# sp-nitech/diffsptk

Measured on AMD Instinct MI355X. Metric: frames/sec STFT->mcep (fl=400 fp=80 nfft=512 M=24), higher is better.
Workload: dtype f32; 1 GPU; BASELINE configs[4] per-GPU shard: STFT->mcep forward, 1024 utterances x 1 s @ 16 kHz per GPU (204800 frames), alpha=0.42 n_iter=10; N=8 is the full 8192-utterance batch; features all-gathered over RCCL when N>1; utterances_per_gpu=1024, global_batch=1024, parallelism=dp1, rccl_world_size=1, reserved_cus=0, gather_depth=0, streams=1

## Files before the change

### diffsptk_amd/csrc/f16_split.h

```cpp
#pragma once

#include "common.h"
#include "mcep_solve.h"

namespace dsa {

typedef _Float16 f16x8 __attribute__((ext_vector_type(8)));
typedef _Float16 f16x4 __attribute__((ext_vector_type(4)));
typedef float f32x2v __attribute__((ext_vector_type(2)));
typedef _Float16 f16x2 __attribute__((ext_vector_type(2)));
typedef const __attribute__((address_space(1))) f16x8* gf16x8_ptr;
typedef int i32x4v __attribute__((ext_vector_type(4)));
__device__ __forceinline__ __amdgpu_buffer_rsrc_t image_rsrc(const _Float16* base, int bytes)
{
    return __builtin_amdgcn_make_buffer_rsrc(const_cast<_Float16*>(base), 0, bytes, 0x00020000);
}
__device__ __forceinline__ f16x8 gload8(__amdgpu_buffer_rsrc_t rsrc, unsigned lane_bytes, int const_bytes)
{
    const i32x4v r = __builtin_amdgcn_raw_buffer_load_b128(rsrc, (int)lane_bytes, const_bytes, 0);
    return __builtin_bit_cast(f16x8, r);
}
typedef const __attribute__((address_space(1))) float* gf32_ptr;

namespace mh {
using namespace mm;
constexpr float SD = 16.f;
constexpr float SM = 1024.f;
constexpr float SE = 65536.f;
constexpr int SE_LOG2 = 16;
constexpr float SG = 4096.f;
constexpr float SL = 128.f;
constexpr int IMG_D = 16 * 64 * 8, IMG_E = 24 * 64 * 8, IMG_G = 16 * 64 * 8;
constexpr int IMG_DH = 0, IMG_DL = IMG_DH + IMG_D, IMG_EH = IMG_DL + IMG_D, IMG_EL = IMG_EH + IMG_E;
constexpr int IMG_GH = IMG_EL + IMG_E, IMG_GL = IMG_GH + IMG_G, IMG_HALVES = IMG_GL + IMG_G;
constexpr int IMG_BYTES = IMG_HALVES * 2 + 32 * 4;
constexpr int EMAX_LOG2 = 15;
constexpr int DH_OFF = 0;
constexpr int DL_OFF = DH_OFF + 16 * 64 * 4;
constexpr int EH_OFF = DL_OFF + 16 * 64 * 4;
constexpr int EL_OFF = EH_OFF + 24 * 64 * 4;
}

namespace mhb {
using namespace mh;
constexpr int IMG_EB = 16 * 2 * 64 * 8, IMG_DB = 2 * 8 * 64 * 8, IMG_GB = 16 * 64 * 8;
constexpr int B_BASE = IMG_BYTES / 2;
constexpr int IMG_EBH = B_BASE, IMG_EBL = IMG_EBH + IMG_EB;
constexpr int IMG_DBH = IMG_EBL + IMG_EB, IMG_DBL = IMG_DBH + IMG_DB;
constexpr int IMG_GBH = IMG_DBL + IMG_DB, IMG_GBL = IMG_GBH + IMG_GB;
constexpr int IMG_B_HALVES = IMG_GBL + IMG_GB;
constexpr int TAIL_B = 32 + 64 + 256;
constexpr int IMG_B_BYTES = IMG_B_HALVES * 2 + TAIL_B * 4;
}

namespace mrh {
constexpr int WAVES = 4;
constexpr int LOG2_SD = 9;
constexpr int LOG2_SE = 16;
constexpr int EMAX_LOG2 = 13;
constexpr int stage_halves(int ks1, int nt) { return (4 * ks1 + 2 * nt) * 512; }
}

__device__ __forceinline__ f32x4 mfma_h(f16x8 a, f16x8 b, f32x4 c)
{
    return __builtin_amdgcn_mfma_f32_16x16x32_f16(a, b, c, 0, 0, 0);
}

__device__ __forceinline__ void split2(float x0, float x1, f16x2& hi, f16x2& lo)
{
    hi = __builtin_convertvector(f32x2v{x0, x1}, f16x2);
    const unsigned hb = __builtin_bit_cast(unsigned, hi);
    unsigned lb;
    asm("v_fma_mixlo_f16 %0, %1, -1.0, %2 op_sel_hi:[1,0,0]\n\ts_nop 0\n\t"
        "v_fma_mixhi_f16 %0, %1, -1.0, %3 op_sel:[1,0,0] op_sel_hi:[1,0,0]\n\ts_nop 0"
        : "=&v"(lb) : "v"(hb), "v"(x0), "v"(x1));
    lo = __builtin_bit_cast(f16x2, lb);
}
__device__ __forceinline__ void split4(float x0, float x1, float x2, float x3, f16x2& hiA, f16x2& hiB, f16x2& loA, f16x2& loB)
{
    hiA = __builtin_convertvector(f32x2v{x0, x1}, f16x2);
    hiB = __builtin_convertvector(f32x2v{x2, x3}, f16x2);
    const unsigned ha = __builtin_bit_cast(unsigned, hiA), hb = __builtin_bit_cast(unsigned, hiB);
    unsigned la, lb;
    asm("v_fma_mixlo_f16 %0, %2, -1.0, %4 op_sel_hi:[1,0,0]\n\t"
        "v_fma_mixlo_f16 %1, %3, -1.0, %6 op_sel_hi:[1,0,0]\n\t"
        "v_fma_mixhi_f16 %0, %2, -1.0, %5 op_sel:[1,0,0] op_sel_hi:[1,0,0]\n\t"
        "v_fma_mixhi_f16 %1, %3, -1.0, %7 op_sel:[1,0,0] op_sel_hi:[1,0,0]\n\ts_nop 0"
        : "=&v"(la), "=&v"(lb) : "v"(ha), "v"(hb), "v"(x0), "v"(x1), "v"(x2), "v"(x3));
    loA = __builtin_bit_cast(f16x2, la);
    loB = __builtin_bit_cast(f16x2, lb);
}
#ifdef DSA_MCEP_NOPK
__device__ __forceinline__ f32x2v fma2(f32x2v c, float s, f32x2v b)
{
    float r0 = __builtin_fmaf(c[0], s, b[0]), r1 = __builtin_fmaf(c[1], s, b[1]);
    asm volatile("" : "+v"(r0));
    return f32x2v{r0, r1};
}
#else
__device__ __forceinline__ f32x2v fma2(f32x2v c, float s, f32x2v b) { return c * f32x2v{s, s} + b; }
#endif
__device__ __forceinline__ f32x2v lo2(f32x4 v) { return __builtin_shufflevector(v, v, 0, 1); }
__device__ __forceinline__ f32x2v hi2(f32x4 v) { return __builtin_shufflevector(v, v, 2, 3); }

__device__ __forceinline__ void split1(float x, _Float16& hi, _Float16& lo)
{
    hi = (_Float16)x;
    lo = (_Float16)(x - (float)hi);
}

__device__ __forceinline__ void split8(const float (&v)[8], f16x8& hi, f16x8& lo)
{
#pragma unroll
    for (int i = 0; i < 8; i += 2) {
        f16x2 h, l;
        split2(v[i], v[i + 1], h, l);
        hi[i] = h[0]; hi[i + 1] = h[1];
        lo[i] = l[0]; lo[i + 1] = l[1];
    }
}

}
```

### diffsptk_amd/csrc/mcep_mfma_f16.h

```cpp
#pragma once

#include <type_traits>

#include "common.h"
#include "f16_split.h"
#include "mcep_solve.h"
#include "pk_math.h"

namespace dsa {

struct StftIn {
    const float* x;
    long Tlen, N;
    int P, left;
    const float* w;
    const float* twiddle;
    float eps;
    float* X_out;
    int pad_mode;
    int zmean;
    float floor_lin;
};

namespace mh {
constexpr float STOP_TAU = 0x1p-20f;
constexpr float STOP_FACTOR = 16.f;
constexpr int H_UPREV = 56;
static_assert(H_UPREV > 48 && H_UPREV < RS, "u_prev sits in the unused tail of the frame's rt window");
constexpr int H_E48 = EL_OFF + 24 * 64 * 4;
constexpr int H_E256 = H_E48 + 256;
constexpr int H_D256 = H_E256 + 52;
constexpr int H_AV = H_D256 + 32;
constexpr int H_NAV = H_AV + 28;
constexpr int H_ZERO = H_NAV + 28;
constexpr int H_WAVE = H_ZERO + 28;
constexpr int h_lds_floats(int waves) { return H_WAVE + waves * WAVE_FLOATS; }
constexpr int FU_LC = 400;
constexpr int FU_NR = (FU_LC + 31) / 32;
constexpr int FU_S = 272;
constexpr int FU_T256 = 0;
constexpr int FU_WTAB = FU_T256 + 512;
constexpr int FU_TWS = FU_WTAB + 2 * 16 * FU_NR;
constexpr int FU_FLOATS = FU_TWS + 256;
static_assert(4 * 272 * 2 == WAVE_FLOATS, "a wave's rt / rr windows double as the STFT tile of four frames");
static_assert(FU_TWS % 4 == 0 && H_WAVE % 4 == 0 && WAVE_FLOATS % 4 == 0, "16-byte aligned LDS tables");
constexpr int h_lds_floats_fused(int waves) { return h_lds_floats(waves) + FU_FLOATS; }
}

#ifndef DSA_FUSED_PK_MASK
#define DSA_FUSED_PK_MASK 31
#endif
#ifndef DSA_FUSED_DBG
#define DSA_FUSED_DBG 0
#endif
template <bool PK> __device__ __forceinline__ v2f fu_mul(v2f a, v2f b) { if constexpr (PK) return pk_mul(a, b); else return sc_mul(a, b); }
template <bool PK> __device__ __forceinline__ v2f fu_cmul(v2f a, v2f t) { if constexpr (PK) return pk_cmul(a, t); else return sc_cmul(a, t); }
template <bool PK, bool ZT> __device__ __forceinline__ void fu_fft16(v2f (&v)[16]) { if constexpr (PK) pk_fft16_il<ZT>(v); else sc_fft16<ZT>(v); }

__global__ __launch_bounds__(256) void mcep_h_prep_kernel(const float* __restrict__ G, const float* __restrict__ D,
                                                          const float* __restrict__ E, _Float16* __restrict__ img)
{
    using namespace mh;
    constexpr float kNeg2Log2e = -2.885390081777926815f, kLn2 = 0.693147180559945309f;
    const int idx = blockIdx.x * 256 + threadIdx.x;
    const int i = idx & 7, l = (idx >> 3) & 63;
    if (idx < IMG_D) {
        const int mt = idx >> 9;
        const int k = 8 * (l >> 4) + i;
        const float v = k < M1 ? (kNeg2Log2e * SD) * D[k * K + mt * 16 + (l & 15)] : 0.f;
        split1(v, img[IMG_DH + idx], img[IMG_DL + idx]);
    } else if (idx < IMG_D + IMG_E) {
        const int e = idx - IMG_D;
        const int j = (e >> 9) & 7, it = e >> 12;
        const int bin = 32 * j + 16 * (i >> 2) + 4 * (l >> 4) + (i & 3);
        const float v = SE * E[bin * M2 + it * 16 + (l & 15)];
        split1(v, img[IMG_EH + e], img[IMG_EL + e]);
    } else if (idx < IMG_D + IMG_E + IMG_G) {
        const int e = idx - IMG_D - IMG_E;
        const int j = (e >> 9) & 7, it = e >> 12;
        const int bin = 32 * j + 16 * (i >> 2) + 4 * (l >> 4) + (i & 3);
        const int coef = it * 16 + (l & 15);
        const float v = coef < M1 ? (kLn2 * SG) * G[bin * M1 + coef] : 0.f;
        split1(v, img[IMG_GH + e], img[IMG_GL + e]);
    }
    if (idx < 32) reinterpret_cast<float*>(img + IMG_HALVES)[idx] = idx < M1 ? G[H * M1 + idx] : 0.f;
}

__device__ __forceinline__ void store_mc_row(float* row, int g, const float (&mcv)[8])
{
    if (g < 3) {
        *reinterpret_cast<f32x4_u4*>(row + 8 * g) = f32x4_u4{mcv[0], mcv[1], mcv[2], mcv[3]};
        *reinterpret_cast<f32x4_u4*>(row + 8 * g + 4) = f32x4_u4{mcv[4], mcv[5], mcv[6], mcv[7]};
    } else {
        row[24] = mcv[0];
    }
}

template <int WAVES, bool FUSED = false, bool HIST_RT = false, bool PADM = false>
__global__ __launch_bounds__(WAVES * 64, WAVES / 4) DSA_PK_TARGET void mcep_mfma_fwd_kernel_h(
    const float* __restrict__ X, long F, int n_iter, const float* __restrict__ G,
    const float* __restrict__ D, const float* __restrict__ E, const float* __restrict__ av,
    float* __restrict__ mc_out, float* __restrict__ hist, long ntiles16, long tiles_shared,
    unsigned int* __restrict__ queue, const _Float16* __restrict__ img, StftIn sti, float* __restrict__ hist_rt, int tail_wgs, float tau)
{
    using namespace mh;
    constexpr float kNeg2Log2e = -2.885390081777926815f, kLn2 = 0.693147180559945309f;
    constexpr float kInvSDM = 1.f / (SD * SM);
    extern __shared__ __attribute__((aligned(16))) float lds[];
    const int tid = threadIdx.x;
    const int lane = tid & 63, wave = tid >> 6;
    const int n = lane & 15, g = lane >> 4;

    {
        const f32x4* src = reinterpret_cast<const f32x4*>(img);
        f32x4* dst = reinterpret_cast<f32x4*>(lds + DH_OFF);
        for (int idx = tid; idx < (2 * IMG_D + 2 * IMG_E) / 8; idx += WAVES * 64) dst[idx] = src[idx];
    }
    {
        const int t2 = tid & 255;
        int r = t2 & 3, gg = (t2 >> 2) & 3, mt = t2 >> 4;
        lds[H_E48 + t2] = E[(mt * 16 + gg * 4 + r) * M2 + 48];
    }
    if (tid < 48) lds[H_E256 + tid] = SE * E[H * M2 + tid];
    if (tid == 48) lds[H_E256 + 48] = E[H * M2 + 48];
    if (tid == 50) lds[H_E256 + 50] = tau;
    if (tid < 32) lds[H_D256 + tid] = tid < M1 ? kNeg2Log2e * D[tid * K + H] : 0.f;
    if (tid < 28) {
        const float a_ = tid < M1 ? av[tid] : 0.f;
        lds[H_AV + tid] = a_;
        lds[H_NAV + tid] = -a_;
        lds[H_ZERO + tid] = 0.f;
    }
    if (FUSED) {
        float* fu = lds + h_lds_floats(WAVES);
        v2f* t256w = reinterpret_cast<v2f*>(fu + FU_T256);
        v2f* wtabw = reinterpret_cast<v2f*>(fu + FU_WTAB);
        v2f* twsw = reinterpret_cast<v2f*>(fu + FU_TWS);
        if (tid < 256) {
            const int m = 2 * (tid & 15) * (tid >> 4);
            t256w[tid] = v2f{0.5f * sti.twiddle[2 * m], 0.5f * sti.twiddle[2 * m + 1]};
        } else if (tid < 256 + 16 * FU_NR) {
            const int i = tid - 256;
            const int l = 2 * (i / FU_NR) + 32 * (i % FU_NR);
            wtabw[i] = v2f{l < FU_LC ? sti.w[l] : 0.f, l + 1 < FU_LC ? sti.w[l + 1] : 0.f};
        }
        if (tid < 128) {
            const int k = 2 * (tid >> 1) + 1 + (tid & 1);
            twsw[tid] = v2f{sti.twiddle[2 * k], sti.twiddle[2 * k + 1]};
        }
    }
    __syncthreads();

    float* rt_lds = lds + H_WAVE + wave * WAVE_FLOATS + n * RS;
    float* rr_lds = rt_lds + 16 * RS;
    int lane_a = lane, lane_b = lane + EL_OFF / 4;
    asm volatile("" : "+v"(lane_a), "+v"(lane_b));
    const f16x8* DH = reinterpret_cast<const f16x8*>(lds + DH_OFF) + lane_a;
    const f16x8* DL = reinterpret_cast<const f16x8*>(lds + DL_OFF) + lane_a;
    const f16x8* EH = reinterpret_cast<const f16x8*>(lds + EH_OFF) + lane_a;
    const f16x8* EL = reinterpret_cast<const f16x8*>(lds) + lane_b;
    const f32x4* E484 = reinterpret_cast<const f32x4*>(lds + H_E48);
    const long wave_id = (long)blockIdx.x * WAVES + wave;
    const long wave_stride = (long)gridDim.x * WAVES;
    const int nq = lane >> 2, gs = lane & 3;
    const GroupMask gq = make_group_mask(gs);
    const unsigned g_lt3 = g < 3 ? 0xffffffffu : 0u, g_eq0 = g == 0 ? 0xffffffffu : 0u;
    float* rt_q = lds + H_WAVE + wave * WAVE_FLOATS + nq * RS;
    float* rr_q = rt_q + 16 * RS;
#ifdef DSA_MCEP_TIMING
    if (blockIdx.x == 0 && threadIdx.x == 0) g_mcep_stamps[12] = __builtin_readcyclecounter();
#endif

#ifdef DSA_MCEP_TIMING
    int tcount = 0;
#define DSA_STAMP_T(i)                                                                   \
    do {                                                                                 \
        if (blockIdx.x == 0 && threadIdx.x == 0 && tcount == 2) g_mcep_stamps[i] = __builtin_readcyclecounter(); \
    } while (0)
#else
#define DSA_STAMP_T(i)
#endif
#ifdef DSA_MCEP_ABL_ONEWAVE
    const bool abl_idle = wave >= WAVES / 2;
#else
    const bool abl_idle = false;
#endif
#ifdef DSA_MCEP_TIMING
    const unsigned long long slot_t0 = wall_clock64();
    int slot_tiles = 0;
#endif
    for (long tile = abl_idle ? ntiles16 : wave_id; tile < ntiles16;) {
        DSA_STAMP_T(16);
#ifdef DSA_MCEP_TIMING
        if (blockIdx.x == 0 && threadIdx.x == 0 && tcount < 12) { g_mcep_stamps[32 + tcount] = __builtin_readcyclecounter(); g_mcep_stamps[48 + tcount] = (unsigned long long)tile; }
#endif
        const long f_raw = tile * 16 + n;
        const bool f_ok = f_raw < F;
        const long f = f_ok ? f_raw : F - 1;

        f32x4 logx[16];
        float logx256;
        if (!FUSED) {
            const float* xf = X + f * K;
#pragma unroll
            for (int mt = 0; mt < 16; ++mt) {
                const float* p = xf + mt * 16 + 4 * g;
                logx[mt] = f32x4{__log2f(p[0]), __log2f(p[1]), __log2f(p[2]), __log2f(p[3])};
            }
            logx256 = __log2f(xf[H]);
        } else {
            constexpr int PKM = DSA_FUSED_PK_MASK;
            const int j = lane & 15, fl = lane >> 4;
            float* wreg = lds + H_WAVE + wave * WAVE_FLOATS;
            v2f* zbuf = reinterpret_cast<v2f*>(wreg);
            v2f* zf = zbuf + fl * 272;
            const float* fu = lds + h_lds_floats(WAVES);
            v2f raw[FU_NR];
            const int tile16 = __builtin_amdgcn_readfirstlane((int)(tile * 16));
            int fr_ns = (int)sti.N, fr_ts = (int)sti.Tlen;
            asm volatile("" : "+s"(fr_ns), "+s"(fr_ts));
            const bool fr_step = tile16 + 16 <= (int)F && fr_ns >= 4 && fr_ts < (1 << 29);
            unsigned fr_sl = 0u, fr_ub = 0u;
            auto fetch = [&](int p, auto first) __attribute__((always_inline)) {
                if (first() || !fr_step) {
                    int flo = fl;
                    asm volatile("" : "+v"(flo));
                    int fr = tile16 + 4 * p + flo;
                    fr = fr < (int)F ? fr : (int)F - 1;
                    fr_ub = (unsigned)fr / (unsigned)sti.N;
                    fr_sl = ((unsigned)fr - fr_ub * (unsigned)sti.N) * (unsigned)sti.P;
                } else {
                    unsigned n_s = (unsigned)sti.N, p_s = (unsigned)sti.P;
                    asm volatile("" : "+s"(n_s), "+s"(p_s));
                    const unsigned np = n_s * p_s;
                    const unsigned s = fr_sl + 4u * p_s;
                    const bool wrap = s >= np;
                    fr_sl = wrap ? s - np : s;
                    fr_ub = wrap ? fr_ub + 1u : fr_ub;
                }
                const unsigned ub = fr_ub;
                const int start = (int)fr_sl - sti.left;
                const float* xb = sti.x + (unsigned long)ub * (unsigned)sti.Tlen;
                const bool interior = start >= 0 && start + 32 * FU_NR <= (int)sti.Tlen;
                if (__builtin_amdgcn_ballot_w64(!interior) == 0) {
                    const v2f_u4* src = reinterpret_cast<const v2f_u4*>(xb + start + 2 * j);
#pragma unroll
                    for (int m1 = 0; m1 < FU_NR; ++m1) raw[m1] = src[16 * m1];
                } else if (!PADM || sti.pad_mode == (int)DSA_PAD_CONSTANT) {
                    const int s00 = start + 2 * j, tl = (int)sti.Tlen;
#pragma unroll
                    for (int m1 = 0; m1 < FU_NR; ++m1) {
                        const int s0 = s00 + 32 * m1, s1 = s0 + 1;
                        const bool ok0 = (unsigned)s0 < (unsigned)tl, ok1 = (unsigned)s1 < (unsigned)tl;
                        const float a0 = xb[ok0 ? s0 : 0], a1 = xb[ok1 ? s1 : 0];
                        raw[m1] = v2f{ok0 ? a0 : 0.f, ok1 ? a1 : 0.f};
                    }
                } else {
                    const int s00 = start + 2 * j, tl = (int)sti.Tlen, md = sti.pad_mode;
                    auto src = [&](int i) __attribute__((always_inline)) -> int {
                        if ((unsigned)i < (unsigned)tl) return i;
                        if (md == (int)DSA_PAD_REPLICATE) return i < 0 ? 0 : tl - 1;
                        if (md == (int)DSA_PAD_CIRCULAR) {
                            int q = i % tl;
                            return q < 0 ? q + tl : q;
                        }
                        if (tl == 1) return 0;
                        const int period = 2 * (tl - 1);
                        int q = i % period;
                        q = q < 0 ? q + period : q;
                        return q < tl ? q : period - q;
                    };
#pragma unroll
                    for (int m1 = 0; m1 < FU_NR; ++m1) {
                        const int s0 = s00 + 32 * m1;
                        raw[m1] = v2f{xb[src(s0)], xb[src(s0 + 1)]};
                    }
                }
            };
            fetch(0, std::true_type{});
#pragma unroll 1
            for (int p = 0; p < 4; ++p) {
                int jo = j * FU_NR, j1 = j, l4 = lane;
                asm volatile("" : "+v"(jo), "+v"(j1), "+v"(l4));
                const v2f* wtab = reinterpret_cast<const v2f*>(fu + FU_WTAB) + jo;
                const v2f* t256 = reinterpret_cast<const v2f*>(fu + FU_T256) + j1;
                v2f v[16];
                if (PADM && sti.zmean) {
                    bool in0[FU_NR], in1[FU_NR];
#pragma unroll
                    for (int m1 = 0; m1 < FU_NR; ++m1) {
                        in0[m1] = 32 * m1 + 30 < FU_LC || 32 * m1 + 2 * j < FU_LC;
                        in1[m1] = 32 * m1 + 31 < FU_LC || 32 * m1 + 1 + 2 * j < FU_LC;
                        raw[m1] = v2f{in0[m1] ? raw[m1].x : 0.f, in1[m1] ? raw[m1].y : 0.f};
                    }
                    pk_zero_mean<FU_NR>(raw, in0, in1, FU_LC);
                }
#pragma unroll
                for (int m1 = 0; m1 < FU_NR; ++m1) {
                    const bool in0 = 32 * m1 + 30 < FU_LC || 32 * m1 + 2 * j < FU_LC;
                    const bool in1 = 32 * m1 + 31 < FU_LC || 32 * m1 + 1 + 2 * j < FU_LC;
                    v[m1] = fu_mul<(PKM & 1) != 0>(v2f{in0 ? raw[m1].x : 0.f, in1 ? raw[m1].y : 0.f}, wtab[m1]);
                }
#pragma unroll
                for (int m1 = FU_NR; m1 < 16; ++m1) v[m1] = v2f{0.f, 0.f};
                if (p < 3) fetch(p + 1, std::false_type{});
#if DSA_FUSED_DBG & 8
                {
                    v2f vin[16], vs[16];
#pragma unroll
                    for (int i = 0; i < 16; ++i) { vin[i] = v[i]; vs[i] = v[i]; }
                    pk_fft16<true>(v);
                    sc_fft16<true>(vs);
                    int nbad = 0, first = -1;
#pragma unroll
                    for (int i = 0; i < 16; ++i) {
                        const bool b = __builtin_bit_cast(unsigned, v[i].x) != __builtin_bit_cast(unsigned, vs[i].x) ||
                                       __builtin_bit_cast(unsigned, v[i].y) != __builtin_bit_cast(unsigned, vs[i].y);
                        if (b && first < 0) first = i;
                        nbad += b ? 1 : 0;
                    }
                    if (nbad) {
                        v2f vr[16];
#pragma unroll
                        for (int i = 0; i < 16; ++i) vr[i] = vin[i];
                        pk_fft16<true>(vr);
                        unsigned* lg = reinterpret_cast<unsigned*>(hist);
                        const unsigned slot = atomicAdd(lg, 1u);
                        if (slot < 4000) {
                            unsigned hwid, xcc;
                            asm volatile("s_getreg_b32 %0, hwreg(HW_REG_HW_ID)" : "=s"(hwid));
                            asm volatile("s_getreg_b32 %0, hwreg(HW_REG_XCC_ID)" : "=s"(xcc));
                            unsigned* r = lg + 16 + 16 * slot;
                            float pkx = 0, pky = 0, scx = 0, scy = 0, rx = 0, ry = 0;
#pragma unroll
                            for (int i = 0; i < 16; ++i)
                                if (i == first) { pkx = v[i].x; pky = v[i].y; scx = vs[i].x; scy = vs[i].y; rx = vr[i].x; ry = vr[i].y; }
                            r[0] = (unsigned)tile; r[1] = p; r[2] = lane; r[3] = first; r[4] = nbad;
                            r[5] = __builtin_bit_cast(unsigned, pkx); r[6] = __builtin_bit_cast(unsigned, pky);
                            r[7] = __builtin_bit_cast(unsigned, scx); r[8] = __builtin_bit_cast(unsigned, scy);
                            r[9] = __builtin_bit_cast(unsigned, rx); r[10] = __builtin_bit_cast(unsigned, ry);
                            r[11] = hwid; r[12] = xcc; r[13] = wave; r[14] = blockIdx.x; r[15] = 0xabcd0000u;
                        }
#pragma unroll
                        for (int i = 0; i < 16; ++i) v[i] = vs[i];
                    }
                }
#else
                fu_fft16<(PKM & 2) != 0, true>(v);
#endif
                if constexpr ((PKM & 4) != 0) {
#pragma unroll
                    for (int k1 = 0; k1 < 16; k1 += 2) {
                        const v2f ta = t256[k1 * 16], tb = t256[(k1 + 1) * 16];
                        const v2f ma = pk_cmul_m(v[FFT16_OUT(k1)], ta), mb = pk_cmul_m(v[FFT16_OUT(k1 + 1)], tb);
                        zf[k1 * 17 + j] = pk_cmul_f(v[FFT16_OUT(k1)], ta, ma);
                        zf[(k1 + 1) * 17 + j] = pk_cmul_f(v[FFT16_OUT(k1 + 1)], tb, mb);
                    }
                } else {
#pragma unroll
                    for (int k1 = 0; k1 < 16; ++k1) {
                        zf[k1 * 17 + j] = fu_cmul<(PKM & 4) != 0>(v[FFT16_OUT(k1)], t256[k1 * 16]);
                    }
                }
                __builtin_amdgcn_wave_barrier();
#pragma unroll
                for (int i = 0; i < 16; ++i) v[i] = zf[j * 17 + i];
                __builtin_amdgcn_wave_barrier();
                fu_fft16<(PKM & 8) != 0, false>(v);
#pragma unroll
                for (int k0 = 0; k0 < 16; ++k0) {
                    zf[j + 16 * k0 + (k0 < 8 ? 1 : 2)] = v[FFT16_OUT(k0)];
                    if (k0 == 8 && j == 0) zf[129] = v[FFT16_OUT(k0)];
                }
                __builtin_amdgcn_wave_barrier();
                v2f pa[4][2], pb[4][2], z0[4];
#pragma unroll
                for (int q = 0; q < 4; ++q) {
                    const v2f* z = zbuf + q * 272;
                    const v4f a2 = *reinterpret_cast<const v4f*>(z + 2 * lane + 2);
                    const v4f b2 = *reinterpret_cast<const v4f*>(z + 256 - 2 * lane);
                    pa[q][0] = v2f{a2.x, a2.y};
                    pa[q][1] = v2f{a2.z, a2.w};
                    pb[q][1] = v2f{b2.x, b2.y};
                    pb[q][0] = v2f{b2.z, b2.w};
                    z0[q] = z[1];
                }
                const v4f tw2 = reinterpret_cast<const v4f*>(fu + FU_TWS)[l4];
                const v2f twA = v2f{tw2.x, tw2.y}, twB = v2f{tw2.z, tw2.w};
                __builtin_amdgcn_wave_barrier();
                const long fr0 = tile * 16 + 4 * p;
#pragma unroll
                for (int q = 0; q < 4; ++q) {
                    v2f se, sp[2];
                    if constexpr ((PKM & 16) != 0) {
                        const v2f eps2 = v2f{sti.eps, sti.eps};
                        v2f Ee;
                        Ee = pk_lo_pm_hi(z0[q], z0[q]);
                        const v2f S0 = pk_add_conj(pa[q][0], pb[q][0]), S1 = pk_add_conj(pa[q][1], pb[q][1]);
                        const v2f Dd0 = pk_sub_conj(pa[q][0], pb[q][0]), Dd1 = pk_sub_conj(pa[q][1], pb[q][1]);
                        const v2f E4 = pk_mul_s(Ee, v2f{4.f, 4.f});
                        const v2f M0 = pk_cmul_m(Dd0, twA), M1 = pk_cmul_m(Dd1, twB);
                        se = pk_fma_sc(E4, Ee, eps2);
                        const v2f Pp0 = pk_cmul_f(Dd0, twA, M0), Pp1 = pk_cmul_f(Dd1, twB, M1);
                        v2f R0, I0, R1, I1;
                        R0 = pk_lo_pm_hi(S0, Pp0);
                        I0 = pk_hi_mp_lo(S0, Pp0);
                        R1 = pk_lo_pm_hi(S1, Pp1);
                        I1 = pk_hi_mp_lo(S1, Pp1);
                        const v2f f0 = pk_fma_sc(R0, R0, eps2), f1 = pk_fma_sc(R1, R1, eps2);
                        sp[0] = pk_fma(I0, I0, f0);
                        sp[1] = pk_fma(I1, I1, f1);
                    } else {
                    const v2f Ee = v2f{sc_add1(z0[q].x, z0[q].y), sc_sub1(z0[q].x, z0[q].y)};
                    const v2f E4 = v2f{sc_mul1s(Ee.x, 4.f), sc_mul1s(Ee.y, 4.f)};
                    se = v2f{sc_fma1sc(E4.x, Ee.x, sti.eps), sc_fma1sc(E4.y, Ee.y, sti.eps)};
#pragma unroll
                    for (int part = 0; part < 2; ++part) {
                        const v2f S = sc_add_conj(pa[q][part], pb[q][part]);
                        const v2f Dd = sc_sub_conj(pa[q][part], pb[q][part]);
                        const v2f Pp = sc_cmul(Dd, part == 0 ? twA : twB);
                        const v2f R = v2f{sc_add1(S.x, Pp.y), sc_sub1(S.x, Pp.y)};
                        const v2f I = v2f{sc_sub1(S.y, Pp.x), sc_nsub1(S.y, Pp.x)};
                        const v2f s0_ = v2f{sc_fma1sc(R.x, R.x, sti.eps), sc_fma1sc(R.y, R.y, sti.eps)};
                        sp[part] = v2f{sc_fma1(I.x, I.x, s0_.x), sc_fma1(I.y, I.y, s0_.y)};
                    }
                    }
                    if (PADM && sti.floor_lin >= 0.f) {
                        float m = sp[0].x > sp[0].y ? sp[0].x : sp[0].y;
                        m = sp[1].x > m ? sp[1].x : m;
                        m = sp[1].y > m ? sp[1].y : m;
                        m = se.x > m ? se.x : m;
                        m = se.y > m ? se.y : m;
                        const float flv = wave64_max(m) * sti.floor_lin;
                        sp[0] = v2f{sp[0].x > flv ? sp[0].x : flv, sp[0].y > flv ? sp[0].y : flv};
                        sp[1] = v2f{sp[1].x > flv ? sp[1].x : flv, sp[1].y > flv ? sp[1].y : flv};
                        se = v2f{se.x > flv ? se.x : flv, se.y > flv ? se.y : flv};
                    }
                    if (sti.X_out && fr0 + q < F) {
                        float* yr = sti.X_out + (fr0 + q) * K;
                        *reinterpret_cast<v2f_u4*>(yr + 2 * l4 + 1) = v2f{sp[0].x, sp[1].x};
                        *reinterpret_cast<v2f_u4*>(yr + 254 - 2 * l4) = v2f{sp[1].y, sp[0].y};
                        if (lane == 0) {
                            yr[0] = se.x;
                            yr[256] = se.y;
                        }
                    }
                    float* st = wreg + q * FU_S;
                    *reinterpret_cast<v2f_u4*>(st + 2 * lane + 1) = v2f{__log2f(sp[0].x), __log2f(sp[1].x)};
                    *reinterpret_cast<v2f*>(st + 254 - 2 * lane) = v2f{__log2f(sp[1].y), __log2f(sp[0].y)};
                    if (lane == 0) {
                        st[0] = __log2f(se.x);
                        st[256] = __log2f(se.y);
                    }
                }
                __builtin_amdgcn_wave_barrier();
                if ((n >> 2) == p) {
                    const float* st = wreg + (n & 3) * FU_S;
#pragma unroll
                    for (int mt = 0; mt < 16; ++mt) logx[mt] = *reinterpret_cast<const f32x4*>(st + 16 * mt + 4 * g);
                    logx256 = st[256];
                }
                __builtin_amdgcn_wave_barrier();
            }
        }
        DSA_STAMP_T(17);

        float mcv[8];
        {
            const _Float16* imgt = img;
            asm volatile("" : "+s"(imgt));
            typedef const __attribute__((address_space(1))) char* gbyte_ptr;
            const gbyte_ptr gimg = (gbyte_ptr)imgt;
            int lane_o = lane;
            asm volatile("" : "+v"(lane_o));
            const unsigned lane16 = 16u * (unsigned)lane_o, n4 = 4u * ((unsigned)lane_o & 15u);
            constexpr int G_AHEAD = 4;
            f16x8 gh[G_AHEAD][2], gl[G_AHEAD][2];
            auto gload = [&](int j) __attribute__((always_inline)) {
#pragma unroll
                for (int it = 0; it < 2; ++it) {
                    gh[j % G_AHEAD][it] = *(gf16x8_ptr)(gimg + (2 * IMG_GH + 1024 * (it * 8 + j)) + lane16);
                    gl[j % G_AHEAD][it] = *(gf16x8_ptr)(gimg + (2 * IMG_GL + 1024 * (it * 8 + j)) + lane16);
                }
            };
#pragma unroll
            for (int j = 0; j < G_AHEAD; ++j) gload(j);
            float gnyq[2];
#pragma unroll
            for (int it = 0; it < 2; ++it) gnyq[it] = *(gf32_ptr)(gimg + (2 * IMG_HALVES + 64 * it) + n4);
            __builtin_amdgcn_sched_barrier(0);
            f32x4 accG[2] = {f32x4{0, 0, 0, 0}, f32x4{0, 0, 0, 0}};
#pragma unroll
            for (int j = 0; j < 8; ++j) {
                f16x8 lh, ll;
#pragma unroll
                for (int tt = 0; tt < 2; ++tt)
#pragma unroll
                    for (int r = 0; r < 4; r += 2) {
                        f16x2 h, l;
                        split2(logx[2 * j + tt][r] * SL, logx[2 * j + tt][r + 1] * SL, h, l);
                        lh[4 * tt + r] = h[0]; lh[4 * tt + r + 1] = h[1];
                        ll[4 * tt + r] = l[0]; ll[4 * tt + r + 1] = l[1];
                    }
#pragma unroll
                for (int it = 0; it < 2; ++it) {
                    const f16x8 ah = gh[j % G_AHEAD][it], al = gl[j % G_AHEAD][it];
                    accG[it] = mfma_h(al, lh, accG[it]);
                    accG[it] = mfma_h(ah, ll, accG[it]);
                    accG[it] = mfma_h(ah, lh, accG[it]);
                }
                if (j + G_AHEAD < 8) {
                    __builtin_amdgcn_sched_barrier(0);
                    gload(j + G_AHEAD);
                }
                __builtin_amdgcn_sched_barrier(0);
            }
#pragma unroll
            for (int it = 0; it < 2; ++it) {
                const float gv = (kLn2 * SG * SL) * gnyq[it];
                accG[it] = mfma4(keep_if(g_eq0, gv), keep_if(g_eq0, logx256), accG[it]);
                accG[it] *= 1.f / (SG * SL);
            }
#pragma unroll
            for (int it = 0; it < 2; ++it)
#pragma unroll
                for (int r = 0; r < 4; ++r) rt_lds[it * 16 + 4 * g + r] = accG[it][r];
            __builtin_amdgcn_wave_barrier();
#pragma unroll
            for (int i = 0; i < 8; ++i) mcv[i] = rt_lds[8 * g + i];
            __builtin_amdgcn_wave_barrier();
        }
        if (!(DSA_FUSED_DBG & 8) && hist && f_ok) store_mc_row(hist + f * M1, g, mcv);

        DSA_STAMP_T(18);
        long tile_next;
        {
            unsigned int nxt = 0;
            if (lane == 0) nxt = atomicAdd(queue, 1u);
            tile_next = wave_stride + (long)__builtin_amdgcn_readfirstlane((int)nxt);
            if (tile_next >= tiles_shared) {
                tile_next = ntiles16;
                if ((tail_wgs > 0 ? (int)blockIdx.x < tail_wgs : wave < WAVES / 2) && tiles_shared < ntiles16) {
                    if (lane == 0) nxt = atomicAdd(queue + 1, 1u);
                    tile_next = tiles_shared + (long)__builtin_amdgcn_readfirstlane((int)nxt);
                }
            }
        }
        unsigned frozen = 0u;
        rt_lds[H_UPREV] = 0.f;
        for (int iter = 0; iter < n_iter; ++iter) {
            DSA_STAMPS_DECL;
            DSA_STAMP(0);
#if DSA_FUSED_DBG & 1
            f32x4 accB[3] = {logx[0], logx[1], logx[2]};
            if (lane == (lane & 15)) accB[0][0] += 65536.f * 4096.f;
            float rt48 = logx256;
            const int back = 0;
#else
            f16x8 bh, bl;
#pragma unroll
            for (int i = 0; i < 8; i += 2) {
                f16x2 h, l;
                split2(mcv[i] * SM, mcv[i + 1] * SM, h, l);
                bh[i] = h[0]; bh[i + 1] = h[1];
                bl[i] = l[0]; bl[i + 1] = l[1];
            }
            float d256 = 0.f;
#pragma unroll
            for (int i = 0; i < 8; ++i) d256 = __builtin_fmaf(mcv[i], lds[H_D256 + 8 * g + i], d256);
            d256 = rows_sum4(d256);
            const float t256 = logx256 + d256;
            DSA_STAMP(6);
#define DSA_SB() __builtin_amdgcn_sched_barrier(0x0004)
            const f32x4 zero4 = {0.f, 0.f, 0.f, 0.f};
            f32x4 tt[16];
            float tmax = t256;
            {
                f16x8 al[4], ah[4];
#pragma unroll
                for (int i = 0; i < 4; ++i) { al[i] = DL[i * 64]; ah[i] = DH[i * 64]; }
                f32x4 c[4] = {zero4, zero4, zero4, zero4}, pc[4] = {zero4, zero4, zero4, zero4};
#pragma unroll
                for (int q = 0; q < 5; ++q) {
                    const bool pm = q < 4, vw = q > 0;
                    f16x8 ah_n[4] = {ah[0], ah[1], ah[2], ah[3]};
#pragma unroll
                    for (int i = 0; i < 4; ++i) {
                        if (q < 3) ah_n[i] = DH[(4 * q + 4 + i) * 64];
                        if (pm) c[i] = mfma_h(al[i], bh, zero4);
                        DSA_SB();
                        if (vw) tt[4 * q - 4 + i] = f32x4{0.f, 0.f, 0.f, 0.f};
                        if (vw) {
                            const f32x2v ta = fma2(lo2(pc[i]), kInvSDM, lo2(logx[4 * q - 4 + i]));
                            const f32x2v tb = fma2(hi2(pc[i]), kInvSDM, hi2(logx[4 * q - 4 + i]));
                            tt[4 * q - 4 + i] = f32x4{ta[0], ta[1], tb[0], tb[1]};
                        }
                        DSA_SB();
                    }
#pragma unroll
                    for (int i = 0; i < 4; ++i) {
                        if (pm) c[i] = mfma_h(ah[i], bl, c[i]);
                        if (q < 3) al[i] = DL[(4 * q + 4 + i) * 64];
                        DSA_SB();
                        if (vw) {
                            const f32x4 v = tt[4 * q - 4 + i];
                            tmax = __builtin_fmaxf(__builtin_fmaxf(tmax, v[0]), v[1]);
                            tmax = __builtin_fmaxf(__builtin_fmaxf(tmax, v[2]), v[3]);
                        }
                        DSA_SB();
                    }
#pragma unroll
                    for (int i = 0; i < 4; ++i) {
                        if (pm) c[i] = mfma_h(ah[i], bh, c[i]);
                        DSA_SB();
                    }
#pragma unroll
                    for (int i = 0; i < 4; ++i) { pc[i] = c[i]; ah[i] = ah_n[i]; }
                }
            }
            DSA_STAMP(7);
            f16x8 eah[3], eal[3];
#pragma unroll
            for (int it = 0; it < 3; ++it) { eah[it] = EH[(it * 8) * 64]; eal[it] = EL[(it * 8) * 64]; }
            tmax = rows_max4(tmax);
            const float mi = __builtin_ceilf(tmax);
            const float sh = (float)EMAX_LOG2 - mi;
            const int back = (int)mi - EMAX_LOG2;
            DSA_STAMP(8);

            const float e256 = __builtin_amdgcn_exp2f(t256 + sh);
            f32x4 accB[3];
#pragma unroll
            for (int it = 0; it < 3; ++it) accB[it] = *reinterpret_cast<const f32x4*>(lds + H_E256 + it * 16 + 4 * g) * e256;
            const float rt48n = e256 * lds[H_E256 + 48];
            f32x2v rt48v = {0.f, 0.f};
            float rt48 = 0.f;
            f16x8 eh_p = {}, el_p = {};
            DSA_SB();
#pragma unroll
            for (int j = 0; j < 9; ++j) {
                f16x8 eh = eh_p, el = el_p;
                f16x8 eah_n[3] = {eah[0], eah[1], eah[2]};
                f32x4 c48[2] = {zero4, zero4};
                if (j < 8) {
                    c48[0] = E484[(2 * j) * 4 + g];
                    c48[1] = E484[(2 * j + 1) * 4 + g];
                }
                if (j > 0 && j < 8) {
#pragma unroll
                    for (int it = 0; it < 3; ++it) eah_n[it] = EH[(it * 8 + j) * 64];
                }
                auto prodE = [&](int i) __attribute__((always_inline)) {
                    if (j > 0) {
                        const int it = i % 3, term = i / 3;
                        accB[it] = mfma_h(term == 0 ? eal[it] : eah[it], term == 1 ? el_p : eh_p, accB[it]);
                    }
                };
                f32x2v ta[2], tb[2];
                float e[2][4];
                auto vecA = [&](int t_) __attribute__((always_inline)) {
                    const f32x4 v = tt[(2 * j + t_) & 15];
                    ta[t_] = lo2(v) + f32x2v{sh, sh};
                    tb[t_] = hi2(v) + f32x2v{sh, sh};
                };
                auto vecB = [&](int t_) __attribute__((always_inline)) {
                    e[t_][0] = __builtin_amdgcn_exp2f(ta[t_][0]);
                    e[t_][1] = __builtin_amdgcn_exp2f(ta[t_][1]);
                };
                auto vecC = [&](int t_) __attribute__((always_inline)) {
                    e[t_][2] = __builtin_amdgcn_exp2f(tb[t_][0]);
                    e[t_][3] = __builtin_amdgcn_exp2f(tb[t_][1]);
                };
                auto vecD = [&](int t_) __attribute__((always_inline)) {
                    rt48v = f32x2v{e[t_][0], e[t_][1]} * lo2(c48[t_]) + rt48v;
                    rt48v = f32x2v{e[t_][2], e[t_][3]} * hi2(c48[t_]) + rt48v;
                };
                auto vecE = [&](int t_, int r) __attribute__((always_inline)) {
                    f16x2 h, l;
                    split2(e[t_][r], e[t_][r + 1], h, l);
                    eh[4 * t_ + r] = h[0]; eh[4 * t_ + r + 1] = h[1];
                    el[4 * t_ + r] = l[0]; el[4 * t_ + r + 1] = l[1];
                };
                const bool vw = j < 8;
                prodE(0); DSA_SB(); if (vw) { vecA(0); vecB(0); } DSA_SB();
                prodE(1); DSA_SB(); if (vw) { vecC(0); vecA(1); } DSA_SB();
                if (j == 8) rt48 = rows_sum4(rt48v[0] + rt48v[1]) + rt48n;
                prodE(2);
                if (j > 0 && j < 8) {
#pragma unroll
                    for (int it = 0; it < 3; ++it) eal[it] = EL[(it * 8 + j) * 64];
                }
                DSA_SB(); if (vw) { vecD(0); vecB(1); } DSA_SB();
                auto vecE4 = [&](int t_) __attribute__((always_inline)) {
                    f16x2 h0, h1, l0, l1;
                    split4(e[t_][0], e[t_][1], e[t_][2], e[t_][3], h0, h1, l0, l1);
                    eh[4 * t_] = h0[0]; eh[4 * t_ + 1] = h0[1]; eh[4 * t_ + 2] = h1[0]; eh[4 * t_ + 3] = h1[1];
                    el[4 * t_] = l0[0]; el[4 * t_ + 1] = l0[1]; el[4 * t_ + 2] = l1[0]; el[4 * t_ + 3] = l1[1];
                };
                if constexpr (FUSED) {
                    prodE(3); DSA_SB(); if (vw) vecE4(0); DSA_SB();
// ... 195 lines not shown
```

### diffsptk_amd/csrc/mcep_solve.h

```cpp
#pragma once

#include <utility>

#include "common.h"

namespace dsa {

typedef float f32x4 __attribute__((ext_vector_type(4)));
typedef float f32x4_u4 __attribute__((ext_vector_type(4), aligned(4)));

namespace mm {
constexpr int H = 256, K = 257;
constexpr int M1 = 25, M2 = 49;
constexpr int KS = 7;
constexpr int NR = 7;
constexpr int RS = 68;
constexpr int DT_OFF = 0;
constexpr int ET_OFF = DT_OFF + 16 * 2 * 64 * 4;
constexpr int E48_OFF = ET_OFF + 3 * 16 * 64 * 4;
constexpr int E256_OFF = E48_OFF + 256;
constexpr int D256_OFF = E256_OFF + 52;
constexpr int AV_OFF = D256_OFF + 28;
constexpr int WAVE_OFF = AV_OFF + 28;
constexpr int WAVE_FLOATS = 2 * 16 * RS;
constexpr int LDS_FLOATS = WAVE_OFF + 4 * WAVE_FLOATS;
}

__device__ __forceinline__ f32x4 mfma4(float a, float b, f32x4 c)
{
    return __builtin_amdgcn_mfma_f32_16x16x4f32(a, b, c, 0, 0, 0);
}

#ifdef DSA_MCEP_TIMING
__device__ unsigned long long g_mcep_stamps[64];
__device__ unsigned long long g_mcep_slotlog[2048 * 3];
#define DSA_STAMPS_DECL unsigned dsa_st_[12] = {0, 0, 0, 0, 0, 0, 0, 0, 0, 0, 0, 0}
#define DSA_STAMP(i) dsa_st_[i] = (unsigned)__builtin_readcyclecounter()
#define DSA_STAMPS_FLUSH                                                                \
    do {                                                                               \
        if (blockIdx.x == 0 && threadIdx.x == 0 && tile == 0 && iter == 1)             \
            for (int i_ = 0; i_ < 12; ++i_) g_mcep_stamps[i_] = dsa_st_[i_];            \
    } while (0)
#else
#define DSA_STAMPS_DECL
#define DSA_STAMP(i)
#define DSA_STAMPS_FLUSH
#endif

struct GroupMask {
    unsigned m[4];
    unsigned gt[4];
};
__device__ __forceinline__ GroupMask make_group_mask(int g)
{
    GroupMask q;
#pragma unroll
    for (int i = 0; i < 4; ++i) {
        q.m[i] = g == i ? 0xffffffffu : 0u;
        q.gt[i] = g > i ? 0xffffffffu : 0u;
    }
    return q;
}
__device__ __forceinline__ float sel4(const GroupMask& q, float c0, float c1, float c2, float c3)
{
    unsigned r = (__float_as_uint(c0) & q.m[0]) | (__float_as_uint(c1) & q.m[1]) | (__float_as_uint(c2) & q.m[2]) |
                 (__float_as_uint(c3) & q.m[3]);
    return __uint_as_float(r);
}
__device__ __forceinline__ float keep_if(unsigned mask, float v) { return __uint_as_float(__float_as_uint(v) & mask); }
__device__ __forceinline__ float rcp_nr(float x)
{
    float r = __builtin_amdgcn_rcpf(x);
    return r * __builtin_fmaf(-x, r, 2.f);
}

__device__ __forceinline__ float rows_sum4(float x)
{
    auto a = __builtin_amdgcn_permlane16_swap(__float_as_uint(x), __float_as_uint(x), false, false);
    x = __uint_as_float(a[0]) + __uint_as_float(a[1]);
    auto b = __builtin_amdgcn_permlane32_swap(__float_as_uint(x), __float_as_uint(x), false, false);
    return __uint_as_float(b[0]) + __uint_as_float(b[1]);
}
__device__ __forceinline__ float rows_max4(float x)
{
    auto a = __builtin_amdgcn_permlane16_swap(__float_as_uint(x), __float_as_uint(x), false, false);
    x = __builtin_fmaxf(__uint_as_float(a[0]), __uint_as_float(a[1]));
    auto b = __builtin_amdgcn_permlane32_swap(__float_as_uint(x), __float_as_uint(x), false, false);
    return __builtin_fmaxf(__uint_as_float(b[0]), __uint_as_float(b[1]));
}
__device__ __forceinline__ unsigned rows_maxu4(unsigned x)
{
    auto a = __builtin_amdgcn_permlane16_swap(x, x, false, false);
    x = a[0] > a[1] ? a[0] : a[1];
    auto b = __builtin_amdgcn_permlane32_swap(x, x, false, false);
    return b[0] > b[1] ? b[0] : b[1];
}

template <int Q>
__device__ __forceinline__ float quad_bcast(float v)
{
    return __int_as_float(__builtin_amdgcn_mov_dpp(__float_as_int(v), Q * 0x55, 0xf, 0xf, true));
}

namespace colm {
using namespace mm;
constexpr int row_len(int i) { return 7 - (i >> 2); }
constexpr int row_off(int i)
{
    int o = 0;
    for (int q = 0; q < i; ++q) o += row_len(q);
    return o;
}
constexpr int TOTAL = row_off(M1);
}
#define COL_AT(a, i, c) (a)[colm::row_off(i) + (c) - ((i) >> 2)]

template <int i>
__device__ __forceinline__ void col_build_rows(float (&a)[colm::TOTAL], const float* rt0, const float* rr0,
                                               const float* avs, const float* rhs2, int gs, const GroupMask& gq)
{
    using namespace mm;
    if constexpr (i < M1) {
        const float* rt_g = rt0 + gs;
        const float* rr_g = rr0 + 27 - gs;
#pragma unroll
        for (int c = i >> 2; c < 6; ++c) COL_AT(a, i, c) = rt_g[i + 4 * c] + rr_g[i - 4 * c];
        const float v24 = rt_g[i + 24] + rr_g[i - 24];
        const float r1 = rt0[i] - avs[i];
        const float r2 = rhs2 ? rhs2[i] : 0.f;
        COL_AT(a, i, 6) = sel4(gq, v24, r1, r2, 0.f);
        col_build_rows<i + 1>(a, rt0, rr0, avs, rhs2, gs, gq);
    }
}

template <int i>
__device__ __forceinline__ void col_build_rows_p(float (&a)[colm::TOTAL], const float* rt0, const float* rr0,
                                                 const float* pa6, const float* pb6, int gs)
{
    using namespace mm;
    if constexpr (i < M1) {
        const float* rt_g = rt0 + gs;
        const float* rr_g = rr0 + 27 - gs;
#pragma unroll
        for (int c = i >> 2; c < 6; ++c) COL_AT(a, i, c) = rt_g[i + 4 * c] + rr_g[i - 4 * c];
        COL_AT(a, i, 6) = pa6[i] + pb6[i];
        col_build_rows_p<i + 1>(a, rt0, rr0, pa6, pb6, gs);
    }
}

template <int Q>
__device__ __forceinline__ void fmac_quad_bcast(float& acc, float s0, float s1)
{
    if constexpr (Q == 0)
        asm volatile("v_fmac_f32_dpp %0, %1, %2 quad_perm:[0,0,0,0] row_mask:0xf bank_mask:0xf" : "+v"(acc) : "v"(s0), "v"(s1));
    else if constexpr (Q == 1)
        asm volatile("v_fmac_f32_dpp %0, %1, %2 quad_perm:[1,1,1,1] row_mask:0xf bank_mask:0xf" : "+v"(acc) : "v"(s0), "v"(s1));
    else if constexpr (Q == 2)
        asm volatile("v_fmac_f32_dpp %0, %1, %2 quad_perm:[2,2,2,2] row_mask:0xf bank_mask:0xf" : "+v"(acc) : "v"(s0), "v"(s1));
    else
        asm volatile("v_fmac_f32_dpp %0, %1, %2 quad_perm:[3,3,3,3] row_mask:0xf bank_mask:0xf" : "+v"(acc) : "v"(s0), "v"(s1));
}

template <int k, int i>
__device__ __forceinline__ void col_update_rows(float (&a)[colm::TOTAL], const float (&pneg)[7])
{
    using namespace mm;
    if constexpr (i < M1) {
#pragma unroll
        for (int c = i >> 2; c < 7; ++c) fmac_quad_bcast<(i & 3)>(COL_AT(a, i, c), pneg[(i >> 2) - (k >> 2)], COL_AT(a, k, c));
        col_update_rows<k, i + 1>(a, pneg);
    }
}
template <int k>
__device__ __forceinline__ void col_elim_step(float (&a)[colm::TOTAL])
{
    const float ninv = -__builtin_amdgcn_rcpf(quad_bcast<(k & 3)>(COL_AT(a, k, k >> 2)));
    float pneg[7];
    constexpr int NP = 7 - (k >> 2);
#pragma unroll
    for (int c = 0; c < 7; ++c) pneg[c] = c < NP ? COL_AT(a, k, (c < NP ? c : 0) + (k >> 2)) * ninv : 0.f;
    if constexpr (NP == 7)
        asm volatile("s_nop 1" : "+v"(pneg[0]), "+v"(pneg[1]), "+v"(pneg[2]), "+v"(pneg[3]), "+v"(pneg[4]), "+v"(pneg[5]), "+v"(pneg[6]));
    else if constexpr (NP == 6)
        asm volatile("s_nop 1" : "+v"(pneg[0]), "+v"(pneg[1]), "+v"(pneg[2]), "+v"(pneg[3]), "+v"(pneg[4]), "+v"(pneg[5]));
    else if constexpr (NP == 5)
        asm volatile("s_nop 1" : "+v"(pneg[0]), "+v"(pneg[1]), "+v"(pneg[2]), "+v"(pneg[3]), "+v"(pneg[4]));
    else if constexpr (NP == 4)
        asm volatile("s_nop 1" : "+v"(pneg[0]), "+v"(pneg[1]), "+v"(pneg[2]), "+v"(pneg[3]));
// ... 245 lines not shown
```

Measured before the change: 575.9 million frames/s.

## Stream mcep constant image into LDS asynchronously, overlapped with first STFT tile

The prologue used to copy the D/E image and several small E/D tail tables into LDS with plain loads and stores before a block barrier. Those tail tables are now precomputed into the prepared image, so the whole head is one linear block. Filler waves load it with global_load_lds_dwordx4 during their first tile's STFT pass and signal completion through an LDS counter. The solver waits on that counter before its first iteration, which takes the prologue's latency off the critical path at the cost of spin-wait synchronisation and inline-asm m0 handling.

```diff
diff --git a/diffsptk_amd/csrc/f16_split.h b/diffsptk_amd/csrc/f16_split.h
--- a/diffsptk_amd/csrc/f16_split.h
+++ b/diffsptk_amd/csrc/f16_split.h
@@ -32,7 +32,11 @@
 constexpr float SL = 128.f;
 constexpr int IMG_D = 16 * 64 * 8, IMG_E = 24 * 64 * 8, IMG_G = 16 * 64 * 8;
 constexpr int IMG_DH = 0, IMG_DL = IMG_DH + IMG_D, IMG_EH = IMG_DL + IMG_D, IMG_EL = IMG_EH + IMG_E;
-constexpr int IMG_GH = IMG_EL + IMG_E, IMG_GL = IMG_GH + IMG_G, IMG_HALVES = IMG_GL + IMG_G;
+constexpr int IMG_FT = 256 + 52 + 32;
+constexpr int IMG_TAIL = IMG_EL + IMG_E;
+constexpr int IMG_FILL_BYTES = IMG_TAIL * 2 + IMG_FT * 4;
+constexpr int IMG_GH = IMG_TAIL + 2 * IMG_FT, IMG_GL = IMG_GH + IMG_G, IMG_HALVES = IMG_GL + IMG_G;
+static_assert(IMG_FILL_BYTES % 16 == 0 && (2 * IMG_GH) % 16 == 0, "16-byte pieces: the linear fill, the streamed G image");
 constexpr int IMG_BYTES = IMG_HALVES * 2 + 32 * 4;
 constexpr int EMAX_LOG2 = 15;
 constexpr int DH_OFF = 0;
diff --git a/diffsptk_amd/csrc/mcep_mfma_f16.h b/diffsptk_amd/csrc/mcep_mfma_f16.h
--- a/diffsptk_amd/csrc/mcep_mfma_f16.h
+++ b/diffsptk_amd/csrc/mcep_mfma_f16.h
@@ -33,7 +33,13 @@
 constexpr int H_AV = H_D256 + 32;
 constexpr int H_NAV = H_AV + 28;
 constexpr int H_ZERO = H_NAV + 28;
-constexpr int H_WAVE = H_ZERO + 28;
+constexpr int H_READY = H_ZERO + 28;
+constexpr int H_WAVE = H_READY + 4;
+static_assert(H_AV - H_E48 == IMG_FT && (H_E48 - DH_OFF) * 2 == IMG_TAIL, "the prepared block's head is the LDS layout DH_OFF .. H_AV");
+constexpr int H_FILL_PIECES = (IMG_FILL_BYTES + 1023) / 1024;
+constexpr int H_FILL_LAST_LANES = (IMG_FILL_BYTES - 1024 * (H_FILL_PIECES - 1)) / 16;
+constexpr int H_FILLERS = 4;
+constexpr int H_TAU_PIECE = ((H_E256 + 50 - DH_OFF) * 4) / 1024;
 constexpr int h_lds_floats(int waves) { return H_WAVE + waves * WAVE_FLOATS; }
 constexpr int FU_LC = 400;
 constexpr int FU_NR = (FU_LC + 31) / 32;
@@ -84,6 +90,28 @@
         split1(v, img[IMG_GH + e], img[IMG_GL + e]);
     }
     if (idx < 32) reinterpret_cast<float*>(img + IMG_HALVES)[idx] = idx < M1 ? G[H * M1 + idx] : 0.f;
+    if (idx < IMG_FT) {
+        float v = 0.f;
+        if (idx < 256) {
+            const int r = idx & 3, gg = (idx >> 2) & 3, mt = idx >> 4;
+            v = E[(mt * 16 + gg * 4 + r) * M2 + 48];
+        } else if (idx < 256 + 48) {
+            v = SE * E[H * M2 + (idx - 256)];
+        } else if (idx == 256 + 48) {
+            v = E[H * M2 + 48];
+        } else if (idx >= 256 + 52) {
+            const int c = idx - (256 + 52);
+            v = c < M1 ? kNeg2Log2e * D[c * K + H] : 0.f;
+        }
+        reinterpret_cast<float*>(img + IMG_TAIL)[idx] = v;
+    }
+}
+
+__device__ __forceinline__ void lds_fill16(const void* base, unsigned off, unsigned lds_dst)
+{
+    unsigned keep;
+    asm volatile("s_mov_b32 %0, m0\n\ts_mov_b32 m0, %3\n\ts_nop 0\n\tglobal_load_lds_dwordx4 %1, %2\n\ts_mov_b32 m0, %0"
+                 : "=&s"(keep) : "v"(off), "s"(base), "s"(lds_dst) : "memory");
 }
 
 __device__ __forceinline__ void store_mc_row(float* row, int g, const float (&mcv)[8])
@@ -110,21 +138,16 @@
     const int tid = threadIdx.x;
     const int lane = tid & 63, wave = tid >> 6;
     const int n = lane & 15, g = lane >> 4;
-
-    {
-        const f32x4* src = reinterpret_cast<const f32x4*>(img);
-        f32x4* dst = reinterpret_cast<f32x4*>(lds + DH_OFF);
-        for (int idx = tid; idx < (2 * IMG_D + 2 * IMG_E) / 8; idx += WAVES * 64) dst[idx] = src[idx];
-    }
-    {
-        const int t2 = tid & 255;
-        int r = t2 & 3, gg = (t2 >> 2) & 3, mt = t2 >> 4;
-        lds[H_E48 + t2] = E[(mt * 16 + gg * 4 + r) * M2 + 48];
-    }
-    if (tid < 48) lds[H_E256 + tid] = SE * E[H * M2 + tid];
-    if (tid == 48) lds[H_E256 + 48] = E[H * M2 + 48];
-    if (tid == 50) lds[H_E256 + 50] = tau;
-    if (tid < 32) lds[H_D256 + tid] = tid < M1 ? kNeg2Log2e * D[tid * K + H] : 0.f;
+#ifdef DSA_MCEP_TIMING
+    if (tid == 0 && blockIdx.x < 256) {
+        const unsigned long long c_ = __builtin_readcyclecounter(), w_ = wall_clock64();
+        g_mcep_startlog[8 * blockIdx.x] = c_;
+        g_mcep_startlog[8 * blockIdx.x + 1] = w_;
+        if (blockIdx.x == 0) g_mcep_stamps[15] = c_;
+    }
+    asm volatile("" ::: "memory");
+#endif
+
     if (tid < 28) {
         const float a_ = tid < M1 ? av[tid] : 0.f;
         lds[H_AV + tid] = a_;
@@ -149,7 +172,14 @@
             twsw[tid] = v2f{sti.twiddle[2 * k], sti.twiddle[2 * k + 1]};
         }
     }
+    if (tid == 0) reinterpret_cast<unsigned*>(lds)[H_READY] = 0u;
     __syncthreads();
+#ifdef DSA_MCEP_TIMING
+    if (tid == 0 && blockIdx.x < 256) {
+        g_mcep_startlog[8 * blockIdx.x + 2] = __builtin_readcyclecounter();
+        g_mcep_startlog[8 * blockIdx.x + 3] = wall_clock64();
+    }
+#endif
 
     float* rt_lds = lds + H_WAVE + wave * WAVE_FLOATS + n * RS;
     float* rr_lds = rt_lds + 16 * RS;
@@ -189,11 +219,59 @@
     const unsigned long long slot_t0 = wall_clock64();
     int slot_tiles = 0;
 #endif
+    const int wave_u = __builtin_amdgcn_readfirstlane(wave);
+    auto fill_all = [&]() __attribute__((always_inline)) {
+#ifndef DSA_MCEP_ABL_NOFILL
+        if (wave_u < WAVES - H_FILLERS) return;
+#pragma unroll 1
+        for (int c = wave_u - (WAVES - H_FILLERS); c < H_FILL_PIECES; c += H_FILLERS) {
+            int lane_f = lane;
+            asm volatile("" : "+v"(lane_f));
+            if (lane_f < (c == H_FILL_PIECES - 1 ? H_FILL_LAST_LANES : 64))
+                lds_fill16(reinterpret_cast<const char*>(img) + 1024 * c, 16u * (unsigned)lane_f, (unsigned)(DH_OFF * 4 + 1024 * c));
+        }
+#endif
+    };
+    auto fill_done = [&]() __attribute__((always_inline)) {
+        asm volatile("s_waitcnt vmcnt(0)" ::: "memory");
+        float tau_s = tau;
+        asm volatile("" : "+s"(tau_s));
+        if (wave_u == WAVES - H_FILLERS + H_TAU_PIECE % H_FILLERS && lane == 50) lds[H_E256 + 50] = tau_s;
+        if (wave_u >= WAVES - H_FILLERS && lane == 0)
+            __hip_atomic_fetch_add(reinterpret_cast<unsigned*>(lds) + H_READY, 1u, __ATOMIC_RELAXED, __HIP_MEMORY_SCOPE_WORKGROUP);
+#ifdef DSA_MCEP_TIMING
+        if (tid == 0 && blockIdx.x < 256) {
+            g_mcep_startlog[8 * blockIdx.x + 6] = __builtin_readcyclecounter();
+            g_mcep_startlog[8 * blockIdx.x + 7] = wall_clock64();
+        }
+#endif
+    };
+    auto publish = [&]() __attribute__((always_inline)) {
+        while (__builtin_amdgcn_readfirstlane((int)reinterpret_cast<volatile unsigned*>(lds)[H_READY]) < H_FILLERS) __builtin_amdgcn_s_sleep(1);
+        asm volatile("" ::: "memory");
+#ifdef DSA_MCEP_TIMING
+        if (tid == 0 && blockIdx.x < 256) {
+            g_mcep_startlog[8 * blockIdx.x + 4] = __builtin_readcyclecounter();
+            g_mcep_startlog[8 * blockIdx.x + 5] = wall_clock64();
+        }
+#endif
+    };
+    static_assert(H_FILLERS <= WAVES / 2 && (H_FILL_PIECES + H_FILLERS - 1) / H_FILLERS + FU_NR < 64, "a filling wave's pieces and a pass's samples: within vmcnt");
+    if (abl_idle || wave_id >= ntiles16) {
+        fill_all();
+        fill_done();
+        publish();
+    }
     for (long tile = abl_idle ? ntiles16 : wave_id; tile < ntiles16;) {
         DSA_STAMP_T(16);
 #ifdef DSA_MCEP_TIMING
         if (blockIdx.x == 0 && threadIdx.x == 0 && tcount < 12) { g_mcep_stamps[32 + tcount] = __builtin_readcyclecounter(); g_mcep_stamps[48 + tcount] = (unsigned long long)tile; }
 #endif
+        const bool first_trip = __builtin_amdgcn_readfirstlane((int)(tile < wave_stride)) != 0;
+        if (first_trip) {
+            fill_all();
+            if (!FUSED) fill_done();
+        }
         const long f_raw = tile * 16 + n;
         const bool f_ok = f_raw < F;
         const long f = f_ok ? f_raw : F - 1;
@@ -280,6 +358,7 @@
             fetch(0, std::true_type{});
 #pragma unroll 1
             for (int p = 0; p < 4; ++p) {
+                if (first_trip && p == 0) fill_done();
                 int jo = j * FU_NR, j1 = j, l4 = lane;
                 asm volatile("" : "+v"(jo), "+v"(j1), "+v"(l4));
                 const v2f* wtab = reinterpret_cast<const v2f*>(fu + FU_WTAB) + jo;
@@ -546,6 +625,7 @@
                 }
             }
         }
+        if (first_trip) publish();
         unsigned frozen = 0u;
         rt_lds[H_UPREV] = 0.f;
         for (int iter = 0; iter < n_iter; ++iter) {
diff --git a/diffsptk_amd/csrc/mcep_solve.h b/diffsptk_amd/csrc/mcep_solve.h
--- a/diffsptk_amd/csrc/mcep_solve.h
+++ b/diffsptk_amd/csrc/mcep_solve.h
@@ -34,6 +34,7 @@
 #ifdef DSA_MCEP_TIMING
 __device__ unsigned long long g_mcep_stamps[64];
 __device__ unsigned long long g_mcep_slotlog[2048 * 3];
+__device__ unsigned long long g_mcep_startlog[256 * 8];
 #define DSA_STAMPS_DECL unsigned dsa_st_[12] = {0, 0, 0, 0, 0, 0, 0, 0, 0, 0, 0, 0}
 #define DSA_STAMP(i) dsa_st_[i] = (unsigned)__builtin_readcyclecounter()
 #define DSA_STAMPS_FLUSH                                                                \
```

After: 580.1 million frames/s, median of 6. Within noise of the previous version (+0.7%).
